# homenc/HElib

Measured on NVIDIA H100. Metric: ctxt_mults_per_s, higher is better.
Workload: dtype u64

## Files before the change

helib_b200/csrc/hb_device_v1.cuh:

```cuda
#pragma once
#include <utility>
#include "hb_device.cuh"

#define HB1_RS 17
#define HB1_BS 273

__device__ __forceinline__ void hb_group_sync(int group, int nthreads) {
#ifdef HB_SIM
  cusim::bar_sync(1 + group, nthreads);
#else
  asm volatile("bar.sync %0, %1;" ::"r"(1 + group), "r"(nthreads) : "memory");
#endif
}

__device__ __forceinline__ void hb1_mac128(u64& hi, u64& lo, u64 a, u64 b) {
#ifdef HB_SIM
  hb_mac128(hi, lo, a, b);
#else
  asm("{\n\t.reg .u64 pl, ph;\n\t"
      "mul.lo.u64 pl, %2, %3;\n\t"
      "mul.hi.u64 ph, %2, %3;\n\t"
      "add.cc.u64 %0, %0, pl;\n\t"
      "addc.u64 %1, %1, ph;\n\t}"
      : "+l"(lo), "+l"(hi)
      : "l"(a), "l"(b));
#endif
}


__device__ __forceinline__ u64 hb1_mulwide(unsigned a, unsigned b) {
#ifdef HB_SIM
  return (u64)a * b;
#else
  u64 r; asm("mul.wide.u32 %0, %1, %2;" : "=l"(r) : "r"(a), "r"(b)); return r;
#endif
}
__device__ __forceinline__ u64 hb1_mulhi_approx(u64 a, u64 b) {
  const unsigned alo = (unsigned)a, ahi = (unsigned)(a >> 32), blo = (unsigned)b, bhi = (unsigned)(b >> 32);
  return hb1_mulwide(ahi, bhi) + (u64)__umulhi(alo, bhi) + (u64)__umulhi(ahi, blo);
}
struct Hb1Mod {
  u64 nq, qb, qb2;
  unsigned qt, qsh;
};
#define HB1_MOD(M, P) Hb1Mod M; M.nq = (P).nq; M.qb = (P).qb; M.qb2 = (P).qb + (P).qb; M.qt = (P).qt; M.qsh = (P).qsh
template <bool SP>
__device__ __forceinline__ u64 hb1_shoup4(u64 y, u64 w, u64 ws, const Hb1Mod& M) {
  const u64 hi = hb1_mulhi_approx(y, ws);
  if (SP) {
    const unsigned tl = (unsigned)hi * M.qt;
    const unsigned ylo = (unsigned)y, yhi = (unsigned)(y >> 32), wlo = (unsigned)w, whi = (unsigned)(w >> 32);
    const u64 R = hb1_mulwide(ylo, wlo) - hi;
    const unsigned rhi = (unsigned)(R >> 32) + yhi * wlo + ylo * whi - (tl << M.qsh);
    return ((u64)rhi << 32) | (unsigned)R;
  }
// ... 483 lines not shown
    const u64* src = J.src[it] + rowoff + c0 + c;
    u64* dst = J.dst[it] + rowoff + c0 + c;
    u64 a[16];
    hb1_unroll<16>([&](auto r) { a[r] = src[(size_t)(16 * r + x) << 8]; });
    hb1_r16_fwd<SP>(a, tw1, M);
    hb1_unroll<16>([&](auto r) { T[c * HB1_BS + HB1_RS * r + x] = a[r]; });
    __syncthreads();
    hb1_unroll<16>([&](auto l) { a[l] = T[c * HB1_BS + HB1_RS * x + l]; });
    hb1_r16_fwd<SP>(a, tw2, M);
    hb1_unroll<16>([&](auto l) { dst[(size_t)(16 * x + l) << 8] = a[l]; });
    __syncthreads();
  }
}
template <bool SP>
__global__ void __launch_bounds__(256, 2) k1_inv_cols(const HbPrimeDev* __restrict__ primes, const HB_GRID_CONSTANT Hb1ColsJob J) {
  HB_SMEM_DECL
  u64* T = HB_SMEM;
  const int tid = threadIdx.x;
  const int pi = J.rows.prime[blockIdx.y];
  const HbPrimeDev P = primes[pi];
  const u64 q = P.q; HB1_MOD(M, P);
  const size_t rowoff = (size_t)pi << J.logN;
  const unsigned c0 = blockIdx.x << 4;
  const int c = tid & 15, x = tid >> 4;
  Hb1TwPtr tw1;
  tw1.p[0] = P.iw + 1; tw1.p[1] = P.iw + 2; tw1.p[2] = P.iw + 4; tw1.p[3] = P.iw + 8;
  Hb1TwReg tw2;
  tw2.load([&](int k, int g) { return P.iw[(16 << k) + (x << k) + g]; });
  for (int it = blockIdx.z; it < J.nitems; it += gridDim.z) {
    const u64* src = J.src[it] + rowoff + c0 + c;
    u64* dst = J.dst[it] + rowoff + c0 + c;
    u64 a[16];
    hb1_unroll<16>([&](auto l) { a[l] = src[(size_t)(16 * x + l) << 8]; });
    hb1_r16_inv<SP>(a, tw2, M);
    hb1_unroll<16>([&](auto l) { T[c * HB1_BS + HB1_RS * x + l] = a[l]; });
    __syncthreads();
    hb1_unroll<16>([&](auto r) { a[r] = T[c * HB1_BS + HB1_RS * r + x]; });
    hb1_r16_inv<SP>(a, tw1, M);
    const u64 fm = J.has_scal ? J.scal[blockIdx.y] : P.ninv, fs = J.has_scal ? J.scal_s[blockIdx.y] : P.ninv_s;
    hb1_unroll<16>([&](auto r) {
      const u64 v = hb_mul_shoup(a[r], fm, fs, q);
      const size_t o = (size_t)(16 * r + x) << 8;
      dst[o] = v;
      for (int p = 0; p < J.npeers; p++) J.peer[p][it][rowoff + c0 + c + o] = v;
    });
    __syncthreads();
  }
}

#define HB1C_BS 276
#define HB1_TS (4 * HB1C_BS)
#define HB1_VS 260

struct Hb1ConvJob {
  const HbConvDev* cv;
  int logN, ngroups;
  int nitems;
  const u64* src[HB_MAXB];
  u64* dst[HB_MAXB];
  u64* stats;
  int src_is_y;
  double* frac[HB_MAXB];
};

template <bool SP>
__global__ void __launch_bounds__(640, 1) k1_conv(const HbPrimeDev* __restrict__ primes, const HB_GRID_CONSTANT Hb1ConvJob J) {
  HB_SMEM_DECL
  const HbConvDev* cv = J.cv;
  const int n = cv->n, nt = cv->nt, NG = J.ngroups;
  u64* Y = HB_SMEM;
  i64* Vb = (i64*)(Y + (size_t)n * HB1_TS);
  u64* W = (u64*)(Vb + 4 * HB1_VS);
  const int tid = threadIdx.x;
  const int grp = tid >> 6, gt = tid & 63;
  const int c = gt & 3, x = gt >> 2;
  const unsigned c0 = blockIdx.x << 2;
  const u64* src = J.src[blockIdx.y];
  u64* dst = J.dst[blockIdx.y];

  for (int j = grp; j < n; j += NG) {
    const int pi = cv->src_prime[j];
    const HbPrimeDev P = primes[pi];
    const u64 q = P.q; HB1_MOD(M, P);
    const u64* s = src + ((size_t)pi << J.logN) + c0 + c;
    u64* Yj = Y + (size_t)j * HB1_TS + c * HB1C_BS;
    u64 a[16];
    hb1_unroll<16>([&](auto l) { a[l] = s[(size_t)(16 * x + l) << 8]; });
    if (J.src_is_y) {
      hb1_unroll<16>([&](auto l) { Yj[HB1_RS * x + l] = a[l]; });
      continue;
    }
    {
      Hb1TwPtr tw;
      tw.p[0] = P.iw + 16 + x; tw.p[1] = P.iw + 32 + 2 * x; tw.p[2] = P.iw + 64 + 4 * x; tw.p[3] = P.iw + 128 + 8 * x;
      hb1_r16_inv<SP>(a, tw, M);
    }
    hb1_unroll<16>([&](auto l) { Yj[HB1_RS * x + l] = a[l]; });
    hb_group_sync(grp, 64);
    hb1_unroll<16>([&](auto r) { a[r] = Yj[HB1_RS * r + x]; });
    {
      Hb1TwPtr tw;
      tw.p[0] = P.iw + 1; tw.p[1] = P.iw + 2; tw.p[2] = P.iw + 4; tw.p[3] = P.iw + 8;
      hb1_r16_inv<SP>(a, tw, M);
    }
    const u64 t = cv->tn[j], ts = cv->tn_s[j];
    hb1_unroll<16>([&](auto r) { Yj[HB1_RS * r + x] = hb_mul_shoup(a[r], t, ts, q); });
  }
  __syncthreads();
  for (int e = tid; e < 1024; e += blockDim.x) {
    const int cc = e >> 8, i1 = e & 255;
    double* fr = J.frac[blockIdx.y];
    double f;
    Vb[cc * HB1_VS + i1] = hb_conv_v(cv, Y + cc * HB1C_BS + HB1_RS * (i1 >> 4) + (i1 & 15), HB1_TS, J.stats, fr ? &f : nullptr);
    if (fr) fr[((size_t)i1 << 8) + c0 + cc] = f;
  }
  __syncthreads();
  u64* Wg = W + (size_t)grp * HB1_TS + c * HB1C_BS;
  for (int t = grp; t < nt; t += NG) {
    const int pi = cv->tgt_prime[t];
    const HbPrimeDev P = primes[pi];
    HB1_MOD(M, P);
    const u64* ct = cv->c + (size_t)t * n;
    u64 a[16];
    {
      const u64 negq = cv->negQ[t], posq = cv->Qmod[t];
      hb1_unroll<2>([&](auto h) {
        u64 ahi[8], alo[8];
        hb1_unroll<8>([&](auto r) {
          const i64 v = Vb[c * HB1_VS + 16 * (8 * h + r) + x];
          const u64 m = v >= 0 ? (u64)v : (u64)(-v);
          const u64 f = v >= 0 ? negq : posq;
          if ((m >> 32) == 0) {
            const u64 p0 = hb1_mulwide((unsigned)m, (unsigned)f);
            const u64 p1 = hb1_mulwide((unsigned)m, (unsigned)(f >> 32)) + (p0 >> 32);
            alo[r] = (p1 << 32) | (unsigned)p0; ahi[r] = p1 >> 32;
          } else { alo[r] = m * f; ahi[r] = __umul64hi(m, f); }
        });
        for (int j = 0; j < n; j++) {
          const u64 cj = ct[j];
          const u64* Yj = Y + (size_t)j * HB1_TS + c * HB1C_BS + x + HB1_RS * 8 * h;
          hb1_unroll<8>([&](auto r) { hb1_mac128(ahi[r], alo[r], Yj[HB1_RS * r], cj); });
        }
        hb1_unroll<8>([&](auto r) { a[8 * h + r] = hb_reduce128_lazy(ahi[r], alo[r], P); });
      });
    }
    {
      Hb1TwPtr tw;
      tw.p[0] = P.fw + 1; tw.p[1] = P.fw + 2; tw.p[2] = P.fw + 4; tw.p[3] = P.fw + 8;
      hb1_r16_fwd<SP>(a, tw, M);
    }
    hb_group_sync(grp, 64);
    hb1_unroll<16>([&](auto r) { Wg[HB1_RS * r + x] = a[r]; });
    hb_group_sync(grp, 64);
    hb1_unroll<16>([&](auto l) { a[l] = Wg[HB1_RS * x + l]; });
    {
      Hb1TwPtr tw;
      tw.p[0] = P.fw + 16 + x; tw.p[1] = P.fw + 32 + 2 * x; tw.p[2] = P.fw + 64 + 4 * x; tw.p[3] = P.fw + 128 + 8 * x;
      hb1_r16_fwd<SP>(a, tw, M);
    }
    u64* d = dst + ((size_t)pi << J.logN) + c0 + c;
    hb1_unroll<16>([&](auto l) { d[(size_t)(16 * x + l) << 8] = a[l]; });
  }
}

struct Hb1Conv1Job {
  int logN, ngroups, cq, nitems;
  int src_prime, nt;
  int tgt_prime[HB_MAXROWS];
  u64 qs_mod[HB_MAXROWS];
  unsigned char nored[HB_MAXROWS];
  u64 ninv, ninv_s;
  const u64* src[HB_MAXB];
  u64* dst[HB_MAXB];
};
template <bool SP>
__global__ void __launch_bounds__(640, 1) k1_conv1(const HbPrimeDev* __restrict__ primes, const HB_GRID_CONSTANT Hb1Conv1Job J) {
  HB_SMEM_DECL
  const int NG = J.ngroups, CQ = J.cq, nt = J.nt;
  u64* Y = HB_SMEM;
  u64* W = Y + (size_t)CQ * HB1_TS;
  const int tid = threadIdx.x;
  const int grp = tid >> 6, gt = tid & 63;
  const int c = gt & 3, x = gt >> 2;
  const unsigned c0 = blockIdx.x * 4u * (unsigned)CQ;
  const u64* src = J.src[blockIdx.y];
  u64* dst = J.dst[blockIdx.y];
  const HbPrimeDev PS = primes[J.src_prime];
  for (int qd = grp; qd < CQ; qd += NG) {
    HB1_MOD(M, PS);
    const u64* s = src + ((size_t)J.src_prime << J.logN) + c0 + 4 * qd + c;
    u64* Yq = Y + (size_t)qd * HB1_TS + c * HB1C_BS;
    u64 a[16];
    hb1_unroll<16>([&](auto l) { a[l] = s[(size_t)(16 * x + l) << 8]; });
    {
      Hb1TwPtr tw;
      tw.p[0] = PS.iw + 16 + x; tw.p[1] = PS.iw + 32 + 2 * x; tw.p[2] = PS.iw + 64 + 4 * x; tw.p[3] = PS.iw + 128 + 8 * x;
      hb1_r16_inv<SP>(a, tw, M);
    }
    hb1_unroll<16>([&](auto l) { Yq[HB1_RS * x + l] = a[l]; });
    hb_group_sync(grp, 64);
    hb1_unroll<16>([&](auto r) { a[r] = Yq[HB1_RS * r + x]; });
    {
      Hb1TwPtr tw;
      tw.p[0] = PS.iw + 1; tw.p[1] = PS.iw + 2; tw.p[2] = PS.iw + 4; tw.p[3] = PS.iw + 8;
      hb1_r16_inv<SP>(a, tw, M);
    }
    hb1_unroll<16>([&](auto r) { Yq[HB1_RS * r + x] = hb_mul_shoup(a[r], J.ninv, J.ninv_s, PS.q); });
  }
  __syncthreads();
  const u64 qs_half = (PS.q - 1) >> 1;
  u64* Wg = W + (size_t)grp * HB1_TS + c * HB1C_BS;
  for (int w = grp; w < nt * CQ; w += NG) {
    const int t = w / CQ, qd = w - t * CQ;
    const int pi = J.tgt_prime[t];
    const HbPrimeDev P = primes[pi];
    HB1_MOD(M, P);
    const u64 adj = P.q - J.qs_mod[t];
    const u64* Yq = Y + (size_t)qd * HB1_TS + c * HB1C_BS + x;
    const bool nored = J.nored[t] != 0;
    u64 a[16];
    hb1_unroll<16>([&](auto r) {
      const u64 y = Yq[HB1_RS * r];
      u64 v = nored ? y : y - __umul64hi(y, P.one_s) * P.q;
      if (y > qs_half) v += adj;
      a[r] = v;
    });
    {
      Hb1TwPtr tw;
      tw.p[0] = P.fw + 1; tw.p[1] = P.fw + 2; tw.p[2] = P.fw + 4; tw.p[3] = P.fw + 8;
      hb1_r16_fwd<SP>(a, tw, M);
    }
    hb_group_sync(grp, 64);
    hb1_unroll<16>([&](auto r) { Wg[HB1_RS * r + x] = a[r]; });
    hb_group_sync(grp, 64);
    hb1_unroll<16>([&](auto l) { a[l] = Wg[HB1_RS * x + l]; });
    {
      Hb1TwPtr tw;
      tw.p[0] = P.fw + 16 + x; tw.p[1] = P.fw + 32 + 2 * x; tw.p[2] = P.fw + 64 + 4 * x; tw.p[3] = P.fw + 128 + 8 * x;
      hb1_r16_fwd<SP>(a, tw, M);
    }
    u64* d = dst + ((size_t)pi << J.logN) + c0 + 4 * qd + c;
    hb1_unroll<16>([&](auto l) { d[(size_t)(16 * x + l) << 8] = a[l]; });
  }
}

__device__ __forceinline__ ulonglong2 hb1_ld2(const u64* p) { return *reinterpret_cast<const ulonglong2*>(p); }
__device__ __forceinline__ void hb1_st2(u64* p, u64 x, u64 y) { ulonglong2 v; v.x = x; v.y = y; *reinterpret_cast<ulonglong2*>(p) = v; }
template <int ND>
__global__ void __launch_bounds__(256) k1_ks_inner(const HbPrimeDev* __restrict__ primes, const HB_GRID_CONSTANT HbKsJob J) {
  const int pi = J.rows.prime[blockIdx.y];
  const HbPrimeDev P = primes[pi];
  const size_t o = (size_t)pi * (size_t)J.N + 2 * ((size_t)blockIdx.x * 256 + threadIdx.x);
  ulonglong2 ea[ND], eb[ND];
#pragma unroll
  for (int i = 0; i < ND; i++) { ea[i] = hb1_ld2(J.evk_a[i] + o); eb[i] = hb1_ld2(J.evk_b[i] + o); }
  const int own = J.own_dig[blockIdx.y];
  const u64 sc = J.scal[blockIdx.y];
  const bool rd = J.mode == 0 || sc != 0;
  for (int it = blockIdx.z; it < J.nitems; it += gridDim.z) {
    ulonglong2 d[ND];
#pragma unroll
    for (int i = 0; i < ND; i++) d[i] = hb1_ld2((i == own ? J.own[it] : J.dig[it][i]) + o);
    u64 h0x = 0, l0x = 0, h0y = 0, l0y = 0, h1x = 0, l1x = 0, h1y = 0, l1y = 0;
    if (rd) {
      const ulonglong2 p0 = hb1_ld2(J.out0[it] + o), p1 = hb1_ld2(J.out1[it] + o);
      if (J.mode == 0) { l0x = p0.x; l0y = p0.y; l1x = p1.x; l1y = p1.y; }
      else { hb1_mac128(h0x, l0x, p0.x, sc); hb1_mac128(h0y, l0y, p0.y, sc); hb1_mac128(h1x, l1x, p1.x, sc); hb1_mac128(h1y, l1y, p1.y, sc); }
    }
#pragma unroll
    for (int i = 0; i < ND; i++) {
      hb1_mac128(h0x, l0x, d[i].x, eb[i].x); hb1_mac128(h0y, l0y, d[i].y, eb[i].y);
      hb1_mac128(h1x, l1x, d[i].x, ea[i].x); hb1_mac128(h1y, l1y, d[i].y, ea[i].y);
    }
    hb1_st2(J.out0[it] + o, hb_reduce128(h0x, l0x, P), hb_reduce128(h0y, l0y, P));
    hb1_st2(J.out1[it] + o, hb_reduce128(h1x, l1x, P), hb_reduce128(h1y, l1y, P));
  }
}

struct Hb1TensorJob {
  u64 N;
  HbRows rows;
  int nitems;
  const u64* a0[HB_MAXB]; const u64* a1[HB_MAXB]; const u64* b0[HB_MAXB]; const u64* b1[HB_MAXB];
  u64* o0[HB_MAXB]; u64* o1[HB_MAXB]; u64* o2[HB_MAXB];
};
__global__ void __launch_bounds__(256) k1_tensor(const HbPrimeDev* __restrict__ primes, const HB_GRID_CONSTANT Hb1TensorJob J) {
  const int pi = J.rows.prime[blockIdx.y];
  const HbPrimeDev P = primes[pi];
  const int it = blockIdx.z;
  const size_t o = (size_t)pi * (size_t)J.N + 2 * ((size_t)blockIdx.x * 256 + threadIdx.x);
  const ulonglong2 a0 = hb1_ld2(J.a0[it] + o), a1 = hb1_ld2(J.a1[it] + o), b0 = hb1_ld2(J.b0[it] + o), b1 = hb1_ld2(J.b1[it] + o);
  u64 hx = 0, lx = 0, hy = 0, ly = 0;
  hb1_mac128(hx, lx, a0.x, b1.x); hb1_mac128(hx, lx, a1.x, b0.x);
  hb1_mac128(hy, ly, a0.y, b1.y); hb1_mac128(hy, ly, a1.y, b0.y);
  hb1_st2(J.o0[it] + o, hb_mulmod(a0.x, b0.x, P), hb_mulmod(a0.y, b0.y, P));
  hb1_st2(J.o1[it] + o, hb_reduce128(hx, lx, P), hb_reduce128(hy, ly, P));
// ... 110 lines not shown
```

helib_b200/csrc/hb_engine.cu:

```cuda
#include "hb_device.cuh"
#include "hb_device_v1.cuh"
#include "hb_device_v2.cuh"
#include "hb_device_gen.cuh"
#include "hb_device_prg.cuh"

#include <algorithm>
#include <cmath>
#include <cstdarg>
#include <cstdio>
#include <cstdlib>
#include <cstring>
#include <map>
#include <set>
#include <string>
#include <vector>

#include "../../include/helib_b200.h"

typedef unsigned __int128 u128;

static size_t blk_parts_smem(int nparts) {
  return (2 * HB1_STAGE + 16 * 256 + (nparts - 1) * 16 * 256) * sizeof(u64) + 256 * sizeof(ulonglong2);
}

static thread_local char g_err[512] = "";
static thread_local int g_chunk = HB_MAXB;
static int hb_fail(int code, const char* fmt, ...) {
  va_list ap; va_start(ap, fmt); vsnprintf(g_err, sizeof(g_err), fmt, ap); va_end(ap);
  return code;
}
#define HB_CUDA(x) do { cudaError_t e_ = (x); if (e_ != cudaSuccess) return hb_fail(HB_ERR_CUDA, "%s failed: %s (%s:%d)", #x, cudaGetErrorString(e_), __FILE__, __LINE__); } while (0)
#define HB_TRY(x) do { int r_ = (x); if (r_ != HB_OK) return r_; } while (0)

static inline u64 h_mulmod(u64 a, u64 b, u64 q) { return (u64)((u128)a * b % q); }
static inline u64 h_powmod(u64 a, u64 e, u64 q) {
  u64 r = 1 % q; a %= q;
  while (e) { if (e & 1) r = h_mulmod(r, a, q); a = h_mulmod(a, a, q); e >>= 1; }
  return r;
}
static inline u64 h_shoup(u64 w, u64 q) { return (u64)(((u128)w << 64) / q); }
static bool h_invmod(u64 a, u64 m, u64* out) {
  __int128 t0 = 0, t1 = 1, r0 = m, r1 = a % m;
  while (r1 != 0) { __int128 qq = r0 / r1, t2 = t0 - qq * t1, r2 = r0 - qq * r1; t0 = t1; t1 = t2; r0 = r1; r1 = r2; }
  if (r0 != 1) return false;
  *out = (u64)(((t0 % (__int128)m) + (__int128)m) % (__int128)m);
  return true;
}
static int h_bitlen(u64 x) { int b = 0; while (x) { b++; x >>= 1; } return b; }

struct ConvEntry {
  HbConvDev h;
  HbConvDev* d;
  void* blob;
  const u64* d_t; const u64* d_t_s;
};

struct hb_ctx {
  int device;
  u64 m; size_t N; int logN, log_blk, nprimes;
  std::vector<u64> q, psi;
  std::vector<HbPrimeDev> h_primes;
  HbPrimeDev* d_primes;
  ulonglong2* d_tw;
  cudaStream_t stream; cudaStream_t own_stream; bool stream_external = false;
  std::vector<int> digit_of; int ndigits; std::vector<int> special;
  u64* tmpA; u64* tmpB;
  double* d_frac; void* d_z; unsigned long long* d_max;
  u64* d_stats;
  HbBcastJob* d_bcast = nullptr;
  std::map<std::string, ConvEntry> convs;
  std::vector<hb_poly*> pool;
  size_t bytes; u64 launches;
  cudaEvent_t ev0, ev1;
  size_t max_smem;
  bool force_v0;
  bool conv1;
  int chunk;
  int resident_ctas;
  bool blk_v2;
  struct TmapKey { const void* base; int logN; bool operator<(const TmapKey& o) const { return base != o.base ? base < o.base : logN < o.logN; } };
  std::map<TmapKey, HbTmap*> tmaps;
  std::vector<HbTmap*> tmap_slabs; size_t tmap_used = 0;
  struct Gen {
    bool on = false;
    u64 m = 0, phim = 0, L = 0, d = 0; int logL = 0, log_blk_L = 0;
    u64 L2 = 0; int logL2 = 0, log_blk_L2 = 0;
    int* d_rep = nullptr; int* d_irep = nullptr;
    HbGenPrime* d_gp = nullptr;
    HbPrimeDev* d_primes_cyc = nullptr; HbPrimeDev* d_primes_cyc2 = nullptr;
    void* tab = nullptr;
    double2* d_W = nullptr;
    u64 *w0 = nullptr, *w1 = nullptr, *wt = nullptr;
    u64 *cA = nullptr, *cB = nullptr;
  } gen;
  struct Pw {
    bool ready = false, triv = true;
    std::vector<long> mvec, pvec, bvec, long_prod;
    std::vector<int> cube_to_poly, short_to_long;
    int* d_cube_to_poly = nullptr; int* d_short_to_long = nullptr;
    u64* cube = nullptr;
    u64* rows = nullptr;
  } pw;
  bool profiling;
  struct ProfRec { const char* name; cudaEvent_t a, b; u64 bytes; };
  std::vector<ProfRec> prof_pending;
  struct ProfAgg { std::string name; u64 launches; double ms; u64 bytes; };
  std::vector<ProfAgg> prof;
  u64* prg_start = nullptr; unsigned* prg_off = nullptr; unsigned long long* prg_ticket = nullptr;
  size_t prg_start_cap = 0, prg_off_cap = 0;
  int prg_window = 0;
  std::vector<hb_poly*> ks_a;
  std::vector<hb_poly*> bsgs;
  std::vector<hb_poly*> block;
  std::vector<hb_poly*> ip;
  std::vector<hb_poly*> leaf;
  u64* ssum = nullptr; size_t ssum_cap = 0;
};
struct HbSeedSched {
  HbPrgKey key;
// ... 676 lines not shown
    J.logN = c->logN; J.epi = epi; J.lazy = lazy;
    if (dir < 0) J.epi = v1_cols_ok(c) ? 2 : 0;
    fill_rows(J.rows, idx + r0, nr);
    for (int i = 0; i < nr; i++) if (scal) { J.scal[i] = scal[r0 + i]; J.scal_s[i] = h_shoup(scal[r0 + i], c->q[idx[r0 + i]]); }
    J.nitems = nitems;
    for (int i = 0; i < nitems; i++) { J.src[i] = src[i]; J.dst[i] = dst[i]; if (dst2) J.dst2[i] = dst2[i]; }
    long units = (long)nr * nitems << (n1 - 4);
    dim3 grid((unsigned)std::min<long>(units, c->resident_ctas));
    pre_launch(c);
    const bool sp = all_special(c);
    if (dir > 0) { if (sp) HB_LAUNCH(k1_fwd_blk<true>, grid, dim3(256), smem, c->stream, c->d_primes, J); else HB_LAUNCH(k1_fwd_blk<false>, grid, dim3(256), smem, c->stream, c->d_primes, J); HB_TRY(post_launch(c, epi == 1 ? "k1_fwd_blk_subscale" : (epi == 3 ? "k1_fwd_blk_digits" : "k1_fwd_blk"), (u64)(epi == 1 ? 3 : 2) * nr * nitems * c->N * 8)); }
    else { if (sp) HB_LAUNCH(k1_inv_blk<true>, grid, dim3(256), smem, c->stream, c->d_primes, J); else HB_LAUNCH(k1_inv_blk<false>, grid, dim3(256), smem, c->stream, c->d_primes, J); HB_TRY(post_launch(c, "k1_inv_blk", (u64)2 * nr * nitems * c->N * 8)); }
  }
  return HB_OK;
}
static int launch_blk_parts_v1(hb_ctx* c, int nparts, const u64* const* src, u64* const* dst, u64* const* o2, int nitems,
                               const int32_t* idx, int n, const u64* scal) {
  const int n1 = c->logN - 8;
  const bool sq = nparts == 2;
  for (int r0 = 0; r0 < n; r0 += HB_MAXROWS) {
    int nr = std::min(HB_MAXROWS, n - r0);
    Hb1BlkJob J; memset(&J, 0, sizeof(J));
    J.logN = c->logN; J.epi = 1; J.lazy = 1;
    fill_rows(J.rows, idx + r0, nr);
    for (int i = 0; i < nr; i++) { J.scal[i] = scal[r0 + i]; J.scal_s[i] = h_shoup(scal[r0 + i], c->q[idx[r0 + i]]); }
    J.nitems = nitems;
    for (int i = 0; i < nparts * nitems; i++) { J.src[i] = src[i]; J.dst[i] = dst[i]; }
    if (sq) for (int i = 0; i < nitems; i++) J.dst2[i] = o2[i];
    long units = (long)nr * nitems << (n1 - 4);
    dim3 grid((unsigned)std::min<long>(units, std::max(1, c->resident_ctas / 2)));
    const size_t smem = blk_parts_smem(nparts);
    pre_launch(c);
    const bool sp = all_special(c);
    if (sq) { if (sp) HB_LAUNCH(k1_fwd_blk_square<true>, grid, dim3(256), smem, c->stream, c->d_primes, J); else HB_LAUNCH(k1_fwd_blk_square<false>, grid, dim3(256), smem, c->stream, c->d_primes, J); }
    else { if (sp) HB_LAUNCH(k1_fwd_blk_tensor<true>, grid, dim3(256), smem, c->stream, c->d_primes, J); else HB_LAUNCH(k1_fwd_blk_tensor<false>, grid, dim3(256), smem, c->stream, c->d_primes, J); }
    HB_TRY(post_launch(c, sq ? "k1_fwd_blk_square" : "k1_fwd_blk_tensor", (u64)(sq ? 7 : 12) * nr * nitems * c->N * 8));
  }
  return HB_OK;
}

#define HB_TMAP_SLAB 512
#ifndef HB_SIM
typedef CUresult (*hb_encode_tiled_fn)(CUtensorMap*, CUtensorMapDataType, cuuint32_t, void*, const cuuint64_t*, const cuuint64_t*,
                                       const cuuint32_t*, const cuuint32_t*, CUtensorMapInterleave, CUtensorMapSwizzle,
                                       CUtensorMapL2promotion, CUtensorMapFloatOOBfill);
static hb_encode_tiled_fn hb_encode_tiled() {
  static hb_encode_tiled_fn fn = [] {
    void* p = nullptr; cudaDriverEntryPointQueryResult qr;
    if (cudaGetDriverEntryPoint("cuTensorMapEncodeTiled", &p, cudaEnableDefault, &qr) != cudaSuccess || qr != cudaDriverEntryPointSuccess) p = nullptr;
    return (hb_encode_tiled_fn)p;
  }();
  return fn;
}
#endif
static bool v2_blk_ok(hb_ctx* c) {
  if (!c->blk_v2 || c->force_v0 || c->log_blk != 8 || c->logN - 8 < 4) return false;
#ifndef HB_SIM
  if (!hb_encode_tiled()) return false;
#endif
  return true;
}
static int get_tmaps(hb_ctx* c, const u64* base, const HbTmap** out) {
  hb_ctx::TmapKey key{base, c->logN};
  auto it = c->tmaps.find(key);
  if (it != c->tmaps.end()) { *out = it->second; return HB_OK; }
  if (c->tmap_slabs.empty() || c->tmap_used == HB_TMAP_SLAB) {
    HbTmap* sl = nullptr;
    HB_TRY(ctx_alloc(c, (void**)&sl, sizeof(HbTmap) * 2 * HB_TMAP_SLAB));
    c->tmap_slabs.push_back(sl); c->tmap_used = 0;
  }
  HbTmap* d = c->tmap_slabs.back() + 2 * c->tmap_used++;
  const int n1 = c->logN - 8;
  const u64 N = (u64)1 << c->logN, N1 = (u64)1 << n1, G = (u64)1 << (n1 - 4);
  HbTmap h[2];
#ifdef HB_SIM
  memset(h, 0, sizeof(h));
  h[0].base = (u64*)base; h[0].rank = 4; h[0].swz128 = 0;
  h[0].dim[0] = 256; h[0].dim[1] = G; h[0].dim[2] = 16; h[0].dim[3] = c->nprimes;
  h[0].stride[0] = 1; h[0].stride[1] = 256; h[0].stride[2] = 256 * G; h[0].stride[3] = N;
  h[0].box[0] = 256; h[0].box[1] = 1; h[0].box[2] = 16; h[0].box[3] = 1;
  h[1].base = (u64*)base; h[1].rank = 3; h[1].swz128 = 1;
  h[1].dim[0] = N1; h[1].dim[1] = 256; h[1].dim[2] = c->nprimes;
  h[1].stride[0] = 1; h[1].stride[1] = N1; h[1].stride[2] = N;
  h[1].box[0] = 16; h[1].box[1] = 256; h[1].box[2] = 1;
#else
  const cuuint32_t ones[4] = {1, 1, 1, 1};
  {
    const cuuint64_t dim[4] = {256, G, 16, (cuuint64_t)c->nprimes};
    const cuuint64_t str[3] = {256 * 8, 256 * 8 * G, N * 8};
    const cuuint32_t box[4] = {256, 1, 16, 1};
    CUresult r = hb_encode_tiled()(&h[0], CU_TENSOR_MAP_DATA_TYPE_UINT64, 4, (void*)base, dim, str, box, ones, CU_TENSOR_MAP_INTERLEAVE_NONE,
                                   CU_TENSOR_MAP_SWIZZLE_NONE, CU_TENSOR_MAP_L2_PROMOTION_L2_256B, CU_TENSOR_MAP_FLOAT_OOB_FILL_NONE);
    if (r != CUDA_SUCCESS) return hb_fail(HB_ERR_CUDA, "cuTensorMapEncodeTiled(BLK view) failed: %d", (int)r);
  }
  {
    const cuuint64_t dim[3] = {N1, 256, (cuuint64_t)c->nprimes};
    const cuuint64_t str[2] = {N1 * 8, N * 8};
    const cuuint32_t box[3] = {16, 256, 1};
    CUresult r = hb_encode_tiled()(&h[1], CU_TENSOR_MAP_DATA_TYPE_UINT64, 3, (void*)base, dim, str, box, ones, CU_TENSOR_MAP_INTERLEAVE_NONE,
                                   CU_TENSOR_MAP_SWIZZLE_128B, CU_TENSOR_MAP_L2_PROMOTION_L2_128B, CU_TENSOR_MAP_FLOAT_OOB_FILL_NONE);
    if (r != CUDA_SUCCESS) return hb_fail(HB_ERR_CUDA, "cuTensorMapEncodeTiled(NAT view) failed: %d", (int)r);
  }
#endif
  HB_CUDA(cudaMemcpy(d, h, sizeof(h), cudaMemcpyHostToDevice));
  c->tmaps[key] = d;
  *out = d;
// ... 208 lines not shown
  H.tn = (const u64*)(B + o_tn); H.tn_s = (const u64*)(B + o_tns); H.fmul = (const u64*)(B + o_fm);
  H.c = (const u64*)(B + o_c); H.negQ = (const u64*)(B + o_nq); H.Qmod = (const u64*)(B + o_qm); H.cp = (const u64*)(B + o_cp);
  H.Q = (const u64*)(B + o_Q); H.Qhalf = (const u64*)(B + o_Qh); H.Qj = (const u64*)(B + o_Qj);
  HB_TRY(ctx_alloc(c, (void**)&E.d, sizeof(HbConvDev)));
  HB_CUDA(cudaMemcpy(E.d, &H, sizeof(HbConvDev), cudaMemcpyHostToDevice));
  auto ins = c->convs.emplace(key, E);
  *out = &ins.first->second;
  return HB_OK;
}

static int norm_scratch(hb_ctx* c) {
  if (c->d_frac) return HB_OK;
  HB_TRY(ctx_alloc(c, (void**)&c->d_frac, (size_t)HB_MAXB * c->N * sizeof(double)));
  HB_TRY(ctx_alloc(c, (void**)&c->d_z, (size_t)HB_MAXB * c->N * 2 * sizeof(double)));
  HB_TRY(ctx_alloc(c, (void**)&c->d_max, HB_MAXB * sizeof(unsigned long long)));
  return HB_OK;
}
static int norm_chunk(hb_ctx* c, int nit, double* out) {
  HbNormJob J; J.logN = c->logN; J.npoly = nit; J.frac = c->d_frac; J.z = (double2*)c->d_z; J.maxbits = c->d_max;
  HB_CUDA(cudaMemsetAsync(c->d_max, 0, nit * sizeof(unsigned long long), c->stream));
  unsigned gx = (unsigned)std::max<size_t>(1, c->N / (HB_THREADS * 4));
  pre_launch(c);
  HB_LAUNCH(k_norm_twist, dim3(gx, nit), dim3(HB_THREADS), 0, c->stream, J);
  HB_TRY(post_launch(c, "k_norm_twist", (u64)nit * c->N * 24));
  for (int logd = c->logN - 1; logd >= 0; logd--) {
    pre_launch(c);
    HB_LAUNCH(k_norm_stage, dim3(gx, nit), dim3(HB_THREADS), 0, c->stream, J, logd, logd == 0 ? 1 : 0);
    HB_TRY(post_launch(c, "k_norm_stage", (u64)nit * c->N * 32));
  }
  unsigned long long bits[HB_MAXB];
  HB_CUDA(cudaMemcpyAsync(bits, c->d_max, nit * sizeof(unsigned long long), cudaMemcpyDeviceToHost, c->stream));
  HB_CUDA(cudaStreamSynchronize(c->stream));
  for (int i = 0; i < nit; i++) { double m2; memcpy(&m2, &bits[i], 8); out[i] = std::sqrt(m2); }
  return HB_OK;
}
static int conv_chunk(hb_ctx* c, u64* const* polys, int nit, const int32_t* src, int n, const int32_t* tgt, int nt, u64 p, int src_is_y = 0, bool want_frac = false) {
  HB_TRY(ctx_scratch(c));
  if (want_frac) HB_TRY(norm_scratch(c));
  ConvEntry* E; HB_TRY(get_conv(c, src, n, tgt, nt, p, &E));
  u64* tA[HB_MAXB]; u64* tB[HB_MAXB];
  tmp_ptrs(c, c->tmpA, nit, tA); tmp_ptrs(c, c->tmpB, nit, tB);
  if (src_is_y) { for (int i = 0; i < nit; i++) tA[i] = polys[i]; }
  else HB_TRY(launch_blk(c, -1, (const u64* const*)polys, tA, nit, src, n, 0, nullptr));
  if (v1_cols_ok(c) && c->conv1 && n == 1 && p <= 1 && !src_is_y && !want_frac && nt <= HB_MAXROWS) {
    Hb1Conv1Job J1; memset(&J1, 0, sizeof(J1));
    static const int cq_env = [] { const char* e = getenv("HB_CONV1_CQ"); int v = e ? atoi(e) : 0; return (v == 1 || v == 2 || v == 4) ? v : 0; }();
    const int cq = cq_env ? cq_env : 4, ng = 10;
    J1.logN = c->logN; J1.ngroups = ng; J1.cq = cq; J1.nitems = nit; J1.src_prime = src[0]; J1.nt = nt;
    const u64 qs = c->q[src[0]];
    for (int t = 0; t < nt; t++) { J1.tgt_prime[t] = tgt[t]; J1.qs_mod[t] = qs % c->q[tgt[t]]; J1.nored[t] = (u128)qs <= (u128)7 * c->q[tgt[t]] ? 1 : 0; }
    u64 ninv; if (!h_invmod(c->N % qs, qs, &ninv)) return hb_fail(HB_ERR_BAD_ARG, "N not invertible");
    J1.ninv = ninv; J1.ninv_s = h_shoup(ninv, qs);
    for (int i = 0; i < nit; i++) { J1.src[i] = tA[i]; J1.dst[i] = tB[i]; }
    const size_t smem1 = (size_t)(cq + ng) * HB1_TS * sizeof(u64);
    pre_launch(c);
    if (all_special(c)) HB_LAUNCH(k1_conv1<true>, dim3(64 / cq, nit), dim3(64 * ng), smem1, c->stream, c->d_primes, J1);
    else HB_LAUNCH(k1_conv1<false>, dim3(64 / cq, nit), dim3(64 * ng), smem1, c->stream, c->d_primes, J1);
    return post_launch(c, "k1_conv1", (u64)(n + nt) * nit * c->N * 8);
  }
  if (v1_cols_ok(c)) {
    int ng = 0; double best = -1; size_t smem1 = 0;
    for (int g = 10; g >= 4; g--) {
      size_t sm = ((size_t)(n + g) * HB1_TS + 4 * HB1_VS) * sizeof(u64);
      if (sm > 224 * 1024) continue;
      int by_smem = (int)((227 * 1024) / (sm + 1024)), by_regs = 65536 / (96 * 64 * g);
      int ctas = std::max(1, std::min(std::min(by_smem, by_regs), 2));
      double work = n + 1.4 * nt, slots = (double)((n + g - 1) / g) + 1.4 * ((nt + g - 1) / g);
      double balance = work / (slots * g);
      double warps = std::min(20.0, 2.0 * g * ctas);
      double score = balance * (0.5 + 0.5 * warps / 20.0) * (ctas >= 2 ? 1.15 : 1.0);
      if (score > best) { best = score; ng = g; smem1 = sm; }
    }
    if (ng > 0) {
      Hb1ConvJob J1; memset(&J1, 0, sizeof(J1));
      J1.cv = E->d; J1.logN = c->logN; J1.ngroups = ng; J1.nitems = nit; J1.stats = c->d_stats; J1.src_is_y = src_is_y;
      if (want_frac) for (int i = 0; i < nit; i++) J1.frac[i] = c->d_frac + (size_t)i * c->N;
      for (int i = 0; i < nit; i++) { J1.src[i] = tA[i]; J1.dst[i] = tB[i]; }
      pre_launch(c);
      if (all_special(c)) HB_LAUNCH(k1_conv<true>, dim3(64, nit), dim3(64 * ng), smem1, c->stream, c->d_primes, J1);
      else HB_LAUNCH(k1_conv<false>, dim3(64, nit), dim3(64 * ng), smem1, c->stream, c->d_primes, J1);
      return post_launch(c, "k1_conv", (u64)(n + nt) * nit * c->N * 8);
    }
  }
  const int n1 = c->logN - c->log_blk;
  int lw = logw_cols(c);
  while (lw > 0 && ((size_t)(n + 2) << (n1 + lw)) * sizeof(u64) > c->max_smem) lw--;
  size_t smem = ((size_t)(n + 2) << (n1 + lw)) * sizeof(u64);
  if (smem > c->max_smem) return hb_fail(HB_ERR_UNSUPPORTED, "base conversion tile needs %zu bytes of shared memory", smem);
  HbConvJob J; memset(&J, 0, sizeof(J));
  J.cv = E->d; J.logN = c->logN; J.log_blk = c->log_blk; J.logw = lw; J.nitems = nit; J.stats = c->d_stats; J.src_is_y = src_is_y;
  if (want_frac) for (int i = 0; i < nit; i++) J.frac[i] = c->d_frac + (size_t)i * c->N;
  for (int i = 0; i < nit; i++) { J.src[i] = tA[i]; J.dst[i] = tB[i]; }
  dim3 grid(1u << (c->log_blk - lw), nit);
  pre_launch(c);
  HB_LAUNCH(k_conv, grid, dim3(HB_THREADS), smem, c->stream, c->d_primes, J);
  return post_launch(c, "k_conv", (u64)(n + nt) * nit * c->N * 8);
}

struct PlanScope {
  hb_ctx* c; int logN, log_blk; HbPrimeDev* dp; size_t N;
  PlanScope(hb_ctx* c_, int plan) : c(c_), logN(c_->logN), log_blk(c_->log_blk), dp(c_->d_primes), N(c_->N) {
    if (plan == 0) { c->logN = c->gen.logL; c->log_blk = c->gen.log_blk_L; c->d_primes = c->gen.d_primes_cyc; c->N = c->gen.L; }
    else { c->logN = c->gen.logL2; c->log_blk = c->gen.log_blk_L2; c->d_primes = c->gen.d_primes_cyc2; c->N = c->gen.L2; }
  }
  ~PlanScope() { c->logN = logN; c->log_blk = log_blk; c->d_primes = dp; c->N = N; }
};
static long h_phi(long m) { long r = m, n = m; for (long p = 2; p * p <= n; p++) if (n % p == 0) { while (n % p == 0) n /= p; r -= r / p; } if (n > 1) r -= r / n; return r; }
static long h_gcd(long a, long b) { while (b) { long t = a % b; a = b; b = t; } return a; }
static bool h_isprime_small(long n) { if (n < 2) return false; for (long p = 2; p * p <= n; p++) if (n % p == 0) return false; return true; }
static u64 h_find_primitive_root(u64 q, u64 e) {
  u64 root = 1, n = e;
  for (u64 p = 2; p <= n; p++) {
    if (n % p) continue;
    u64 pp = 1; while (n % p == 0) { n /= p; pp *= p; }
    u64 g = 2;
    for (;; g++) if (h_isprime_small((long)g) && h_powmod(g, (q - 1) / p, q) != 1) break;
    root = h_mulmod(root, h_powmod(g, (q - 1) / pp, q), q);
  }
  return root;
}
static void poly_mul_binom(std::vector<long>& a, long k) { std::vector<long> r(a.size() + k, 0); for (size_t i = 0; i < a.size(); i++) { r[i + k] += a[i]; r[i] -= a[i]; } a.swap(r); }
static void poly_div_binom(std::vector<long>& a, long k) {
  std::vector<long> qv(a.size() - k, 0);
  for (long i = (long)a.size() - 1; i >= k; i--) { long cq = a[i]; qv[i - k] = cq; a[i] -= cq; a[i - k] += cq; }
  a.swap(qv);
}
static int h_mobius(long n) { int mu = 1; for (long p = 2; p * p <= n; p++) if (n % p == 0) { n /= p; if (n % p == 0) return 0; mu = -mu; } if (n > 1) mu = -mu; return mu; }
static std::vector<long> h_cyclotomic(long m) {
  std::vector<long> a(1, 1);
  for (long d = 1; d <= m; d++) if (m % d == 0 && h_mobius(d) == 1) poly_mul_binom(a, m / d);
// ... 2044 lines not shown
```

Baseline: 3074.

## Store base-conversion output tiles through TMA tensor-map bulk stores

The conversion kernels (k1_conv, k1_conv1) now stage each group's 256x4 output tile in shared memory and issue a single 5D cp.async.bulk.tensor store from one thread. This replaces the per-thread strided 8-byte global stores, which hit 32-byte sectors inefficiently. It adds an extra group barrier, a smem transposition pass and a wait on prior bulk reads before the staging buffer is reused. The tensor map is encoded once against tmpB and assumes dst is always tmpB, and a standalone microbenchmark is included to compare store methods.

```diff
diff --git a/bench_micro/ubench_conv_store.cu b/bench_micro/ubench_conv_store.cu
--- /dev/null
+++ b/bench_micro/ubench_conv_store.cu
@@ -0,0 +1,142 @@
+#include <cstdio>
+#include <cstdlib>
+#include <cuda.h>
+#include <cuda_runtime.h>
+typedef unsigned long long u64;
+
+#define LOGN 16
+#define ROWS 19
+#define ITEMS 64
+#define NG 10
+#define NSRC 10
+#define CBS 276
+#define TS (4 * CBS)
+#define SMEM ((NSRC + NG) * TS * 8 + 4 * 260 * 8)
+
+#define CK(x) do { cudaError_t e_ = (x); if (e_ != cudaSuccess) { printf("%s:%d %s\n", __FILE__, __LINE__, cudaGetErrorString(e_)); exit(1); } } while (0)
+
+__device__ __forceinline__ void gsync(int g) { asm volatile("bar.sync %0, 64;" ::"r"(1 + g) : "memory"); }
+__device__ __forceinline__ void fence_async() { asm volatile("fence.proxy.async.shared::cta;" ::: "memory"); }
+__device__ __forceinline__ void wait_read() { asm volatile("cp.async.bulk.wait_group.read 0;" ::: "memory"); }
+__device__ __forceinline__ void wait_all() { asm volatile("cp.async.bulk.wait_group 0;" ::: "memory"); }
+__device__ __forceinline__ void bulk32(u64* g, const u64* s) {
+  asm volatile("cp.async.bulk.global.shared::cta.bulk_group [%0], [%1], 32;" ::"l"(g), "r"((unsigned)__cvta_generic_to_shared(s)) : "memory");
+  asm volatile("cp.async.bulk.commit_group;" ::: "memory");
+}
+__device__ __forceinline__ void tstore2d(const CUtensorMap* m, const u64* s, int c0, int r0) {
+  asm volatile("cp.async.bulk.tensor.2d.global.shared::cta.bulk_group [%0, {%2, %3}], [%1];"
+               ::"l"(m), "r"((unsigned)__cvta_generic_to_shared(s)), "r"(c0), "r"(r0) : "memory");
+  asm volatile("cp.async.bulk.commit_group;" ::: "memory");
+}
+
+enum { S, B, T };
+template <int MODE>
+__global__ void __launch_bounds__(640, 1) kstore(u64* __restrict__ dst, const __grid_constant__ CUtensorMap tm) {
+  extern __shared__ u64 sm[];
+  u64* W = sm + NSRC * TS + 4 * 260;
+  const int tid = threadIdx.x, grp = tid >> 6, gt = tid & 63, c = gt & 3, x = gt >> 2;
+  const unsigned c0 = blockIdx.x << 2;
+  u64* const Wt = W + grp * TS;
+  u64* const Wg = Wt + c * CBS;
+  for (int t = grp; t < ROWS; t += NG) {
+    u64 a[16];
+#pragma unroll
+    for (int r = 0; r < 16; r++) a[r] = ((u64)t << 40) ^ ((u64)blockIdx.x << 20) ^ (u64)(tid * 16 + r);
+    if (MODE != S) wait_read();
+    gsync(grp);
+#pragma unroll
+    for (int r = 0; r < 16; r++) Wg[17 * r + x] = a[r];
+    gsync(grp);
+#pragma unroll
+    for (int l = 0; l < 16; l++) a[l] = Wg[17 * x + l] + 1;
+    const size_t row0 = ((size_t)blockIdx.y * ROWS + t) << 8;
+    if (MODE == S) {
+      u64* d = dst + (row0 << 8) + c0 + c;
+#pragma unroll
+      for (int l = 0; l < 16; l++) d[(size_t)(16 * x + l) << 8] = a[l];
+    } else {
+      gsync(grp);
+#pragma unroll
+      for (int l = 0; l < 16; l++) Wt[4 * (MODE == B ? 17 * x + l : 16 * x + l) + c] = a[l];
+      fence_async();
+      gsync(grp);
+      if (MODE == B) {
+        u64* d = dst + (row0 << 8) + c0;
+#pragma unroll
+        for (int k = 0; k < 4; k++) { const int i = gt + 64 * k; bulk32(d + ((size_t)i << 8), Wt + 4 * (i + (i >> 4))); }
+      } else if (gt == 0) {
+        tstore2d(&tm, Wt, (int)c0, (int)row0);
+      }
+    }
+  }
+  if (MODE != S) wait_all();
+}
+
+__global__ void kstream(u64* __restrict__ dst, size_t n) {
+  for (size_t i = (size_t)blockIdx.x * 256 + threadIdx.x; i < n / 2; i += (size_t)gridDim.x * 256)
+    ((ulonglong2*)dst)[i] = make_ulonglong2(i, i + 1);
+}
+
+typedef CUresult (*encode_fn)(CUtensorMap*, CUtensorMapDataType, cuuint32_t, void*, const cuuint64_t*, const cuuint64_t*,
+                              const cuuint32_t*, const cuuint32_t*, CUtensorMapInterleave, CUtensorMapSwizzle,
+                              CUtensorMapL2promotion, CUtensorMapFloatOOBfill);
+
+static cudaEvent_t e0, e1;
+template <class F> static double time_ms(F&& f) {
+  f(); CK(cudaDeviceSynchronize());
+  float best = 1e30f;
+  for (int rep = 0; rep < 5; rep++) {
+    CK(cudaEventRecord(e0)); f(); CK(cudaEventRecord(e1)); CK(cudaEventSynchronize(e1));
+    float ms; CK(cudaEventElapsedTime(&ms, e0, e1)); if (ms < best) best = ms;
+  }
+  return best;
+}
+
+int main() {
+  int nsm = 0; CK(cudaDeviceGetAttribute(&nsm, cudaDevAttrMultiProcessorCount, 0));
+  cudaDeviceProp prop; CK(cudaGetDeviceProperties(&prop, 0));
+  printf("device: %s, %d SMs\n", prop.name, nsm);
+  const size_t n = (size_t)ITEMS * ROWS << LOGN;
+  const double bytes = (double)n * 8;
+  u64* dst; CK(cudaMalloc(&dst, n * 8));
+  u64* ref; CK(cudaMalloc(&ref, n * 8));
+  CK(cudaEventCreate(&e0)); CK(cudaEventCreate(&e1));
+  void* p = nullptr; cudaDriverEntryPointQueryResult qr;
+  CK(cudaGetDriverEntryPoint("cuTensorMapEncodeTiled", &p, cudaEnableDefault, &qr));
+  if (!p || qr != cudaDriverEntryPointSuccess) { printf("no cuTensorMapEncodeTiled\n"); return 1; }
+  CUtensorMap tm;
+  const cuuint64_t dims[2] = {256, (cuuint64_t)ITEMS * ROWS * 256}, strides[1] = {256 * 8};
+  const cuuint32_t box[2] = {4, 256}, es[2] = {1, 1};
+  CUresult r = ((encode_fn)p)(&tm, CU_TENSOR_MAP_DATA_TYPE_UINT64, 2, dst, dims, strides, box, es, CU_TENSOR_MAP_INTERLEAVE_NONE,
+                              CU_TENSOR_MAP_SWIZZLE_NONE, CU_TENSOR_MAP_L2_PROMOTION_NONE, CU_TENSOR_MAP_FLOAT_OOB_FILL_NONE);
+  if (r != CUDA_SUCCESS) { printf("cuTensorMapEncodeTiled: %d\n", (int)r); return 1; }
+  printf("grid 64 x %d CTAs of %d threads, %d B of shared memory, %.0f MiB written per launch\n", ITEMS, 64 * NG, SMEM, bytes / (1 << 20));
+  const dim3 grid(64, ITEMS), block(64 * NG);
+  CK(cudaFuncSetAttribute(kstore<S>, cudaFuncAttributeMaxDynamicSharedMemorySize, SMEM));
+  CK(cudaFuncSetAttribute(kstore<B>, cudaFuncAttributeMaxDynamicSharedMemorySize, SMEM));
+  CK(cudaFuncSetAttribute(kstore<T>, cudaFuncAttributeMaxDynamicSharedMemorySize, SMEM));
+  const char* names[3] = {"S scalar 8-byte stores", "B 32-byte cp.async.bulk, staged", "T 2D tensor-map store per tile"};
+  for (int m = 0; m < 3; m++) {
+    auto launch = [&] {
+      if (m == S) kstore<S><<<grid, block, SMEM>>>(dst, tm);
+      else if (m == B) kstore<B><<<grid, block, SMEM>>>(dst, tm);
+      else kstore<T><<<grid, block, SMEM>>>(dst, tm);
+      CK(cudaGetLastError());
+    };
+    const double ms = time_ms(launch);
+    int same = 1;
+    if (m == S) CK(cudaMemcpy(ref, dst, n * 8, cudaMemcpyDeviceToDevice));
+    else {
+      CK(cudaMemset(dst, 0, n * 8)); launch(); CK(cudaDeviceSynchronize());
+      u64 *h0 = (u64*)malloc(n * 8), *h1 = (u64*)malloc(n * 8);
+      CK(cudaMemcpy(h0, ref, n * 8, cudaMemcpyDeviceToHost)); CK(cudaMemcpy(h1, dst, n * 8, cudaMemcpyDeviceToHost));
+      for (size_t i = 0; i < n && same; i++) same = h0[i] == h1[i];
+      free(h0); free(h1);
+    }
+    printf("%-34s %7.3f ms  %7.1f GB/s  %s\n", names[m], ms, bytes / (ms * 1e-3) / 1e9, same ? "same output" : "OUTPUT DIFFERS");
+  }
+  const double ms = time_ms([&] { kstream<<<4 * nsm, 256>>>(dst, n); });
+  printf("%-34s %7.3f ms  %7.1f GB/s\n", "streaming write, same bytes", ms, bytes / (ms * 1e-3) / 1e9);
+  printf("%s\n", cudaGetErrorString(cudaGetLastError()));
+  return 0;
+}
diff --git a/helib_b200/csrc/hb_device_v1.cuh b/helib_b200/csrc/hb_device_v1.cuh
--- a/helib_b200/csrc/hb_device_v1.cuh
+++ b/helib_b200/csrc/hb_device_v1.cuh
@@ -1,6 +1,9 @@
 #pragma once
 #include <utility>
 #include "hb_device.cuh"
+#ifndef HB_SIM
+#include <cuda.h>
+#endif
 
 #define HB1_RS 17
 #define HB1_BS 273
@@ -590,6 +593,26 @@
 #define HB1_TS (4 * HB1C_BS)
 #define HB1_VS 260
 
+__device__ __forceinline__ void hb1_conv_store(u64* Wt, u64* d, const void* omap, const u64 (&a)[16], int grp, int gt, unsigned col0,
+                                               int pi, int it) {
+  const int c = gt & 3, x = gt >> 2;
+#ifdef HB_SIM
+  (void)Wt; (void)omap; (void)grp; (void)pi; (void)it;
+  hb1_unroll<16>([&](auto l) { d[((size_t)(16 * x + l) << 8) + col0 + c] = a[l]; });
+#else
+  (void)d;
+  hb_group_sync(grp, 64);
+  hb1_unroll<16>([&](auto l) { Wt[64 * l + 4 * x + c] = a[l]; });
+  hb1_fence_async();
+  hb_group_sync(grp, 64);
+  if (gt == 0) {
+    asm volatile("cp.async.bulk.tensor.5d.global.shared::cta.bulk_group [%0, {%2, %3, %4, %5, %6}], [%1];"
+                 ::"l"(omap), "r"((unsigned)__cvta_generic_to_shared(Wt)), "r"(col0), "r"(0), "r"(0), "r"(pi), "r"(it) : "memory");
+    asm volatile("cp.async.bulk.commit_group;" ::: "memory");
+  }
+#endif
+}
+
 struct Hb1ConvJob {
   const HbConvDev* cv;
   int logN, ngroups;
@@ -599,6 +622,9 @@
   u64* stats;
   int src_is_y;
   double* frac[HB_MAXB];
+#ifndef HB_SIM
+  CUtensorMap omap;
+#endif
 };
 
 template <bool SP>
@@ -614,7 +640,6 @@
   const int c = gt & 3, x = gt >> 2;
   const unsigned c0 = blockIdx.x << 2;
   const u64* src = J.src[blockIdx.y];
-  u64* dst = J.dst[blockIdx.y];
 
   for (int j = grp; j < n; j += NG) {
     const int pi = cv->src_prime[j];
@@ -653,7 +678,8 @@
     if (fr) fr[((size_t)i1 << 8) + c0 + cc] = f;
   }
   __syncthreads();
-  u64* Wg = W + (size_t)grp * HB1_TS + c * HB1C_BS;
+  u64* const Wt = W + (size_t)grp * HB1_TS;
+  u64* const Wg = Wt + c * HB1C_BS;
   for (int t = grp; t < nt; t += NG) {
     const int pi = cv->tgt_prime[t];
     const HbPrimeDev P = primes[pi];
@@ -687,6 +713,7 @@
       tw.p[0] = P.fw + 1; tw.p[1] = P.fw + 2; tw.p[2] = P.fw + 4; tw.p[3] = P.fw + 8;
       hb1_r16_fwd<SP>(a, tw, M);
     }
+    hb1_bulk_wait_read();
     hb_group_sync(grp, 64);
     hb1_unroll<16>([&](auto r) { Wg[HB1_RS * r + x] = a[r]; });
     hb_group_sync(grp, 64);
@@ -696,9 +723,15 @@
       tw.p[0] = P.fw + 16 + x; tw.p[1] = P.fw + 32 + 2 * x; tw.p[2] = P.fw + 64 + 4 * x; tw.p[3] = P.fw + 128 + 8 * x;
       hb1_r16_fwd<SP>(a, tw, M);
     }
-    u64* d = dst + ((size_t)pi << J.logN) + c0 + c;
-    hb1_unroll<16>([&](auto l) { d[(size_t)(16 * x + l) << 8] = a[l]; });
-  }
+#ifdef HB_SIM
+    const void* omap = nullptr;
+#else
+    const void* omap = &J.omap;
+#endif
+    hb1_conv_store(Wt, J.dst[blockIdx.y] + ((size_t)pi << J.logN), omap, a, threadIdx.x >> 6, threadIdx.x & 63, blockIdx.x << 2, pi,
+                   blockIdx.y);
+  }
+  hb1_bulk_wait_all();
 }
 
 struct Hb1Conv1Job {
@@ -710,6 +743,9 @@
   u64 ninv, ninv_s;
   const u64* src[HB_MAXB];
   u64* dst[HB_MAXB];
+#ifndef HB_SIM
+  CUtensorMap omap;
+#endif
 };
 template <bool SP>
 __global__ void __launch_bounds__(640, 1) k1_conv1(const HbPrimeDev* __restrict__ primes, const HB_GRID_CONSTANT Hb1Conv1Job J) {
@@ -747,7 +783,7 @@
   }
   __syncthreads();
   const u64 qs_half = (PS.q - 1) >> 1;
-  u64* Wg = W + (size_t)grp * HB1_TS + c * HB1C_BS;
+  u64* const Wg = W + (size_t)grp * HB1_TS + c * HB1C_BS;
   for (int w = grp; w < nt * CQ; w += NG) {
     const int t = w / CQ, qd = w - t * CQ;
     const int pi = J.tgt_prime[t];
@@ -768,6 +804,7 @@
       tw.p[0] = P.fw + 1; tw.p[1] = P.fw + 2; tw.p[2] = P.fw + 4; tw.p[3] = P.fw + 8;
       hb1_r16_fwd<SP>(a, tw, M);
     }
+    hb1_bulk_wait_read();
     hb_group_sync(grp, 64);
     hb1_unroll<16>([&](auto r) { Wg[HB1_RS * r + x] = a[r]; });
     hb_group_sync(grp, 64);
@@ -777,9 +814,15 @@
       tw.p[0] = P.fw + 16 + x; tw.p[1] = P.fw + 32 + 2 * x; tw.p[2] = P.fw + 64 + 4 * x; tw.p[3] = P.fw + 128 + 8 * x;
       hb1_r16_fwd<SP>(a, tw, M);
     }
-    u64* d = dst + ((size_t)pi << J.logN) + c0 + 4 * qd + c;
-    hb1_unroll<16>([&](auto l) { d[(size_t)(16 * x + l) << 8] = a[l]; });
-  }
+#ifdef HB_SIM
+    const void* omap = nullptr;
+#else
+    const void* omap = &J.omap;
+#endif
+    hb1_conv_store(Y + (size_t)(CQ + (threadIdx.x >> 6)) * HB1_TS, dst + ((size_t)pi << J.logN), omap, a, threadIdx.x >> 6, threadIdx.x & 63, blockIdx.x * 4u * (unsigned)CQ + 4 * qd, pi,
+                   blockIdx.y);
+  }
+  hb1_bulk_wait_all();
 }
 
 __device__ __forceinline__ ulonglong2 hb1_ld2(const u64* p) { return *reinterpret_cast<const ulonglong2*>(p); }
diff --git a/helib_b200/csrc/hb_engine.cu b/helib_b200/csrc/hb_engine.cu
--- a/helib_b200/csrc/hb_engine.cu
+++ b/helib_b200/csrc/hb_engine.cu
@@ -65,6 +65,9 @@
   cudaStream_t stream; cudaStream_t own_stream; bool stream_external = false;
   std::vector<int> digit_of; int ndigits; std::vector<int> special;
   u64* tmpA; u64* tmpB;
+#ifndef HB_SIM
+  CUtensorMap conv_omap; bool conv_omap_ok = false;
+#endif
   double* d_frac; void* d_z; unsigned long long* d_max;
   u64* d_stats;
   HbBcastJob* d_bcast = nullptr;
@@ -847,6 +850,21 @@
   }();
   return fn;
 }
+static int conv_out_map(hb_ctx* c, CUtensorMap* out) {
+  if (!c->conv_omap_ok) {
+    if (!hb_encode_tiled()) return hb_fail(HB_ERR_UNSUPPORTED, "cuTensorMapEncodeTiled is not available: the conversion kernels need it");
+    const cuuint64_t dim[5] = {256, 16, 16, (cuuint64_t)c->nprimes, HB_MAXB};
+    const cuuint64_t str[4] = {16 * 256 * 8, 256 * 8, (cuuint64_t)c->N * 8, (cuuint64_t)c->nprimes * c->N * 8};
+    const cuuint32_t box[5] = {4, 16, 16, 1, 1}, ones[5] = {1, 1, 1, 1, 1};
+    CUresult r = hb_encode_tiled()(&c->conv_omap, CU_TENSOR_MAP_DATA_TYPE_UINT64, 5, (void*)c->tmpB, dim, str, box, ones,
+                                   CU_TENSOR_MAP_INTERLEAVE_NONE, CU_TENSOR_MAP_SWIZZLE_NONE, CU_TENSOR_MAP_L2_PROMOTION_NONE,
+                                   CU_TENSOR_MAP_FLOAT_OOB_FILL_NONE);
+    if (r != CUDA_SUCCESS) return hb_fail(HB_ERR_CUDA, "cuTensorMapEncodeTiled(conversion output view) failed: %d", (int)r);
+    c->conv_omap_ok = true;
+  }
+  *out = c->conv_omap;
+  return HB_OK;
+}
 #endif
 static bool v2_blk_ok(hb_ctx* c) {
   if (!c->blk_v2 || c->force_v0 || c->log_blk != 8 || c->logN - 8 < 4) return false;
@@ -1161,6 +1179,9 @@
     u64 ninv; if (!h_invmod(c->N % qs, qs, &ninv)) return hb_fail(HB_ERR_BAD_ARG, "N not invertible");
     J1.ninv = ninv; J1.ninv_s = h_shoup(ninv, qs);
     for (int i = 0; i < nit; i++) { J1.src[i] = tA[i]; J1.dst[i] = tB[i]; }
+#ifndef HB_SIM
+    HB_TRY(conv_out_map(c, &J1.omap));
+#endif
     const size_t smem1 = (size_t)(cq + ng) * HB1_TS * sizeof(u64);
     pre_launch(c);
     if (all_special(c)) HB_LAUNCH(k1_conv1<true>, dim3(64 / cq, nit), dim3(64 * ng), smem1, c->stream, c->d_primes, J1);
@@ -1185,6 +1206,9 @@
       J1.cv = E->d; J1.logN = c->logN; J1.ngroups = ng; J1.nitems = nit; J1.stats = c->d_stats; J1.src_is_y = src_is_y;
       if (want_frac) for (int i = 0; i < nit; i++) J1.frac[i] = c->d_frac + (size_t)i * c->N;
       for (int i = 0; i < nit; i++) { J1.src[i] = tA[i]; J1.dst[i] = tB[i]; }
+#ifndef HB_SIM
+      HB_TRY(conv_out_map(c, &J1.omap));
+#endif
       pre_launch(c);
       if (all_special(c)) HB_LAUNCH(k1_conv<true>, dim3(64, nit), dim3(64 * ng), smem1, c->stream, c->d_primes, J1);
       else HB_LAUNCH(k1_conv<false>, dim3(64, nit), dim3(64 * ng), smem1, c->stream, c->d_primes, J1);
```

Result: faster. 3112, median of 6 (+1.2%).
